# SHI-Labs/Versatile-Diffusion

Hardware: NVIDIA H100
Metric: 512x512 images/sec @ 50-step DDIM (bs=4/GPU) (higher is better)
Workload: dtype bf16

## Files before the change

### versatile-diffusion_b200/csrc/attention.cu

```cuda
#include "common.cuh"
#include "host_util.h"

namespace vdb {

constexpr int kBQ = 128;
constexpr float kRescaleThreshold = 8.0f;

struct alignas(64) AttnParams {
  CUtensorMap tmQ;
  CUtensorMap tmK;
  CUtensorMap tmV;
  int Nq, Nk;
  int q_bs, kv_bs;
  int q_col0, k_col0;
  int dv;
  int causal;
  float scale_log2;
  __nv_bfloat16* out;
  long long ldo;
};

template <int DK, int DVP, int BKV, int KV_STAGES>
constexpr size_t attention_smem_bytes() {
  return (DK / 64) * kBQ * 128 + KV_STAGES * ((DK / 64) * BKV * 128 + (BKV / 64) * DVP * 128) + (1 + 4 * KV_STAGES) * 8 + 1024;
}

template <int DK, int DVP, int BKV, int KV_STAGES>
__global__ void __launch_bounds__(288, 1) attention_kernel(const __grid_constant__ AttnParams p) {
  constexpr int KA = DK / 64;
  constexpr int KVA = BKV / 64;
  constexpr uint32_t kQBytes = KA * kBQ * 128;
  constexpr uint32_t kKBytes = KA * BKV * 128;
  constexpr uint32_t kVAtom = DVP * 128;
  constexpr uint32_t kVBytes = KVA * kVAtom;
  static_assert(BKV == 64 || BKV == 128, "kv tile");
  static_assert(kVAtom % 1024 == 0, "V atom must keep 1024B alignment");
  static_assert(DVP % 16 == 0 && DVP <= 256, "invalid wgmma N for PV");

  extern __shared__ __align__(1024) uint8_t smem_raw[];
  uint8_t* smem = reinterpret_cast<uint8_t*>((reinterpret_cast<uintptr_t>(smem_raw) + 1023) & ~uintptr_t(1023));
  uint8_t* sQ = smem;
  uint8_t* sK = sQ + kQBytes;
  uint8_t* sV = sK + KV_STAGES * kKBytes;
  uint64_t* q_full = reinterpret_cast<uint64_t*>(sV + KV_STAGES * kVBytes);
  uint64_t* k_full = q_full + 1;
  uint64_t* k_empty = k_full + KV_STAGES;
  uint64_t* v_full = k_empty + KV_STAGES;
  uint64_t* v_empty = v_full + KV_STAGES;

  const int warp = threadIdx.x >> 5;
  const int lane = threadIdx.x & 31;
  const int q0 = blockIdx.x * kBQ;
  const int head = blockIdx.y;
  const int b = blockIdx.z;

  int ntiles = (p.Nk + BKV - 1) / BKV;
  if (p.causal) ntiles = min(ntiles, (q0 + kBQ + BKV - 1) / BKV);

  if (warp == 8 && lane == 0) {
    tma_prefetch_desc(&p.tmQ);
    tma_prefetch_desc(&p.tmK);
    tma_prefetch_desc(&p.tmV);
  }
  if (threadIdx.x == 0) {
    mbar_init(q_full, 1);
    for (int s = 0; s < KV_STAGES; ++s) {
      mbar_init(&k_full[s], 1); mbar_init(&k_empty[s], 8);
      mbar_init(&v_full[s], 1); mbar_init(&v_empty[s], 8);
    }
    fence_barrier_init();
  }
  __syncthreads();
  pdl_launch_dependents();
  pdl_wait();

  if (warp == 8) {
    if (lane == 0) {
      mbar_arrive_expect_tx(q_full, kQBytes);
      for (int a = 0; a < KA; ++a)
        tma_load_2d(sQ + a * kBQ * 128, &p.tmQ, q_full, p.q_col0 + head * DK + a * 64, b * p.q_bs + q0);
      for (int j = 0; j < ntiles; ++j) {
        const int st = j % KV_STAGES;
        const uint32_t ph = (j / KV_STAGES) & 1;
        mbar_wait(&k_empty[st], ph ^ 1);
        mbar_arrive_expect_tx(&k_full[st], kKBytes);
        for (int a = 0; a < KA; ++a)
          tma_load_2d(sK + st * kKBytes + a * BKV * 128, &p.tmK, &k_full[st], p.k_col0 + head * DK + a * 64,
                      b * p.kv_bs + j * BKV);
        mbar_wait(&v_empty[st], ph ^ 1);
        mbar_arrive_expect_tx(&v_full[st], kVBytes);
        for (int a = 0; a < KVA; ++a)
          tma_load_2d(sV + st * kVBytes + a * kVAtom, &p.tmV, &v_full[st], b * p.kv_bs + j * BKV + a * 64, head * DVP);
      }
    }
    return;
  }

  const int g = warp >> 2;
  const int row0 = g * 64 + (warp & 3) * 16 + (lane >> 2);
  const int c2 = 2 * (lane & 3);
  const int q_idx[2] = {q0 + row0, q0 + row0 + 8};
  const int ksteps = (p.dv + 15) / 16;
  float o[DVP / 2];
#pragma unroll
  for (int i = 0; i < DVP / 2; ++i) o[i] = 0.f;
  float m_ref[2] = {-INFINITY, -INFINITY};
  float l_sum[2] = {0.f, 0.f};
  mbar_wait(q_full, 0);
#pragma unroll 1
  for (int j = 0; j < ntiles; ++j) {
    const int st = j % KV_STAGES;
    const uint32_t ph = (j / KV_STAGES) & 1;
    float s[BKV / 2];
    mbar_wait(&k_full[st], ph);
    wgmma_fence();
#pragma unroll
    for (int a = 0; a < KA; ++a) {
      const uint64_t qd = make_desc_sw128(smem_u32(sQ + a * kBQ * 128 + g * 64 * 128));
      const uint64_t kd = make_desc_sw128(smem_u32(sK + st * kKBytes + a * BKV * 128));
#pragma unroll
      for (int k = 0; k < 4; ++k)
        if (a * 4 + k < ksteps)
          wgmma_ss<BKV>(s, qd + 2 * k, kd + 2 * k, (a > 0 || k > 0) ? 1u : 0u);
    }
    wgmma_commit();
    wgmma_wait<0>();
    wgmma_fence_regs(s);
    __syncwarp();
    if (lane == 0) mbar_arrive(&k_empty[st]);

    const int kv0 = j * BKV;
    if (kv0 + BKV > p.Nk || p.causal) {
#pragma unroll
      for (int i = 0; i < 2; ++i) {
        const int lim = p.causal ? min(p.Nk, q_idx[i] + 1) : p.Nk;
#pragma unroll
        for (int jj = 0; jj < BKV / 8; ++jj)
#pragma unroll
          for (int e = 0; e < 2; ++e)
            if (kv0 + 8 * jj + c2 + e >= lim) s[4 * jj + 2 * i + e] = -INFINITY;
      }
    }
    float m_scaled[2];
#pragma unroll
    for (int i = 0; i < 2; ++i) {
      float mx = -INFINITY;
#pragma unroll
      for (int jj = 0; jj < BKV / 8; ++jj) mx = fmaxf(mx, fmaxf(s[4 * jj + 2 * i], s[4 * jj + 2 * i + 1]));
      mx = fmaxf(mx, __shfl_xor_sync(0xffffffffu, mx, 1));
      mx = fmaxf(mx, __shfl_xor_sync(0xffffffffu, mx, 2));
      const float m_new = fmaxf(m_ref[i], mx);
      if (j == 0 || m_ref[i] == -INFINITY) {
        m_ref[i] = m_new;
      } else if ((m_new - m_ref[i]) * p.scale_log2 > kRescaleThreshold) {
        const float factor = ex2_mufu((m_ref[i] - m_new) * p.scale_log2);
        m_ref[i] = m_new;
        l_sum[i] *= factor;
#pragma unroll
        for (int jj = 0; jj < DVP / 8; ++jj) {
          o[4 * jj + 2 * i] *= factor;
          o[4 * jj + 2 * i + 1] *= factor;
        }
      }
      m_scaled[i] = (m_ref[i] == -INFINITY) ? 0.f : m_ref[i] * p.scale_log2;
    }
    uint32_t pa[BKV / 16][4];
#pragma unroll
    for (int kk = 0; kk < BKV / 16; ++kk) {
#pragma unroll
      for (int h = 0; h < 4; ++h) {
        const int i = h & 1;
        const int idx = 8 * kk + 4 * (h >> 1) + 2 * i;
        const float e0 = ex2_mufu(fmaf(s[idx], p.scale_log2, -m_scaled[i]));
        const float e1 = ex2_mufu(fmaf(s[idx + 1], p.scale_log2, -m_scaled[i]));
        l_sum[i] += e0 + e1;
        pa[kk][h] = pack_bf16x2(e0, e1);
      }
    }
    mbar_wait(&v_full[st], ph);
    wgmma_fence();
#pragma unroll
    for (int kk = 0; kk < BKV / 16; ++kk) {
      const uint64_t vd = make_desc_sw128(smem_u32(sV + st * kVBytes + (kk >> 2) * kVAtom));
      wgmma_rs<DVP>(o, pa[kk], vd + 2 * (kk & 3), 1u);
    }
    wgmma_commit();
    wgmma_wait<0>();
    wgmma_fence_regs(o);
    __syncwarp();
    if (lane == 0) mbar_arrive(&v_empty[st]);
  }

#pragma unroll
  for (int i = 0; i < 2; ++i) {
    float l = l_sum[i];
    l += __shfl_xor_sync(0xffffffffu, l, 1);
    l += __shfl_xor_sync(0xffffffffu, l, 2);
    const float inv_l = 1.f / l;
    if (q_idx[i] >= p.Nq) continue;
    __nv_bfloat16* orow = p.out + (static_cast<long long>(b) * p.q_bs + q_idx[i]) * p.ldo + head * p.dv;
#pragma unroll
    for (int jj = 0; jj < DVP / 8; ++jj) {
      const int col = 8 * jj + c2;
      if (col < p.dv)
        *reinterpret_cast<uint32_t*>(orow + col) = pack_bf16x2(o[4 * jj + 2 * i] * inv_l, o[4 * jj + 2 * i + 1] * inv_l);
    }
  }
}

struct AttnArgs {
  const void *Q, *K, *Vt;
  long long ldq, ldk, ldv;
  int B, H, q_bstride, kv_bstride;
};

template <int DK, int DVP, int BKV, int KV_STAGES>
static int launch_attention(AttnParams& p, const AttnArgs& a, cudaStream_t stream) {
  constexpr size_t smem = attention_smem_bytes<DK, DVP, BKV, KV_STAGES>();
  static_assert(smem <= 227 * 1024, "attention smem budget");
  auto kernel = attention_kernel<DK, DVP, BKV, KV_STAGES>;
  static bool configured = false;
  if (!configured) {
    VDB_CUDA_CHECK(cudaFuncSetAttribute(kernel, cudaFuncAttributeMaxDynamicSharedMemorySize, static_cast<int>(smem)));
    prefer_max_smem(kernel);
    configured = true;
  }
  int rc = make_tmap_2d(&p.tmQ, a.Q, static_cast<uint64_t>(a.ldq), static_cast<uint64_t>(a.B) * a.q_bstride, a.ldq * 2, 64, kBQ);
  if (rc) return rc;
  rc = make_tmap_2d(&p.tmK, a.K, static_cast<uint64_t>(a.ldk), static_cast<uint64_t>(a.B) * a.kv_bstride, a.ldk * 2, 64, BKV);
  if (rc) return rc;
  rc = make_tmap_2d(&p.tmV, a.Vt, static_cast<uint64_t>(a.B) * a.kv_bstride, static_cast<uint64_t>(a.H) * DVP, a.ldv * 2, 64, DVP);
  if (rc) return rc;
  dim3 grid((p.Nq + kBQ - 1) / kBQ, a.H, a.B);
  VDB_CUDA_CHECK(launch_pdl(kernel, grid, dim3(288), smem, stream, p));
  count_launch();
  return VDB_OK;
}

}

using namespace vdb;

extern "C" {

int vdb_attention_dk_pad(int d_head) { return d_head <= 64 ? 64 : (d_head <= 128 ? 128 : (d_head <= 192 ? 192 : -1)); }
int vdb_attention_dv_pad(int d_head) {
  if (d_head <= 48) return 48;
  if (d_head <= 64) return 64;
  if (d_head <= 80) return 80;
  if (d_head <= 160) return 160;
  return -1;
}

int vdb_attention_bf16(const void* Q, long long ldq, int q_col0, const void* K, long long ldk, int k_col0,
                       const void* Vt, long long ldv, void* out, long long ldo, int B, int H, int Nq, int Nk,
                       int q_bstride, int kv_bstride, int d_head, float scale, int causal, void* stream) {
  if (!Q || !K || !Vt || !out || B <= 0 || H <= 0 || Nq <= 0 || Nk <= 0)
    return set_error(VDB_ERR_INVALID, "attention: null/empty argument");
  const int DK = vdb_attention_dk_pad(d_head), DVP = vdb_attention_dv_pad(d_head);
  if (DK < 0 || DVP < 0) return set_error(VDB_ERR_UNSUPPORTED, "attention: d_head %d not supported (<= 160)", d_head);
  if ((d_head % 8) || (ldo % 8) || (ldq % 8) || (ldk % 8) || (ldv % 8))
    return set_error(VDB_ERR_INVALID, "attention: d_head and leading dims must be multiples of 8");
  if (q_bstride <= 0) q_bstride = Nq;
  if (kv_bstride <= 0) kv_bstride = Nk;
  if (q_bstride < Nq || kv_bstride < Nk || (kv_bstride % 8))
    return set_error(VDB_ERR_INVALID, "attention: need q_bstride >= Nq, kv_bstride >= Nk and kv_bstride %% 8 == 0 (got %d, %d)",
                     q_bstride, kv_bstride);
  AttnParams p;
  memset(&p, 0, sizeof(p));
  const AttnArgs a{Q, K, Vt, ldq, ldk, ldv, B, H, q_bstride, kv_bstride};
  p.Nq = Nq; p.Nk = Nk; p.q_bs = q_bstride; p.kv_bs = kv_bstride; p.q_col0 = q_col0; p.k_col0 = k_col0; p.dv = d_head; p.causal = causal;
  p.scale_log2 = scale * 1.4426950408889634f;
  p.out = reinterpret_cast<__nv_bfloat16*>(out);
  p.ldo = ldo;
  cudaStream_t st = reinterpret_cast<cudaStream_t>(stream);
  if (DK == 64 && DVP == 48) return launch_attention<64, 48, 128, 2>(p, a, st);
  if (DK == 64 && DVP == 64) return launch_attention<64, 64, 128, 2>(p, a, st);
  if (DK == 128 && DVP == 80) return launch_attention<128, 80, 128, 2>(p, a, st);
  if (DK == 192 && DVP == 160) return launch_attention<192, 160, 64, 2>(p, a, st);
  return set_error(VDB_ERR_UNSUPPORTED, "attention: no kernel for d_head %d", d_head);
}

}
```

### versatile-diffusion_b200/csrc/common.cuh

```cuda
#pragma once
#include <cuda.h>
#include <cuda_bf16.h>
#include <cuda_runtime.h>
#include <stdint.h>

namespace vdb {

#define VDB_DEVINL __device__ __forceinline__

enum : int {
  VDB_OK = 0,
  VDB_ERR_INVALID = 1,
  VDB_ERR_CUDA = 2,
  VDB_ERR_UNSUPPORTED = 3,
};

VDB_DEVINL float4 lds_f4(uint32_t addr) {
  float4 v;
  asm volatile("ld.shared.v4.f32 {%0, %1, %2, %3}, [%4];" : "=f"(v.x), "=f"(v.y), "=f"(v.z), "=f"(v.w) : "r"(addr));
  return v;
}

VDB_DEVINL uint32_t smem_u32(const void* p) {
  return static_cast<uint32_t>(__cvta_generic_to_shared(p));
}

VDB_DEVINL uint32_t lane_id() {
  uint32_t l;
  asm volatile("mov.u32 %0, %%laneid;" : "=r"(l));
  return l;
}

VDB_DEVINL bool elect_one() {
  uint32_t pred = 0;
  asm volatile(
      "{\n\t"
      ".reg .pred P;\n\t"
      "elect.sync _|P, 0xffffffff;\n\t"
      "selp.u32 %0, 1, 0, P;\n\t"
      "}\n"
      : "=r"(pred));
  return pred != 0;
}

VDB_DEVINL void mbar_init(uint64_t* bar, uint32_t count) {
  asm volatile("mbarrier.init.shared::cta.b64 [%0], %1;" ::"r"(smem_u32(bar)), "r"(count));
}
VDB_DEVINL void fence_barrier_init() {
  asm volatile("fence.mbarrier_init.release.cluster;" ::: "memory");
}
VDB_DEVINL void fence_proxy_async_smem() {
  asm volatile("fence.proxy.async.shared::cta;" ::: "memory");
}
VDB_DEVINL void mbar_arrive_expect_tx(uint64_t* bar, uint32_t bytes) {
  asm volatile("mbarrier.arrive.expect_tx.shared::cta.b64 _, [%0], %1;" ::"r"(smem_u32(bar)),
               "r"(bytes)
               : "memory");
}
VDB_DEVINL void mbar_arrive(uint64_t* bar) {
  asm volatile("mbarrier.arrive.shared::cta.b64 _, [%0];" ::"r"(smem_u32(bar)) : "memory");
}
VDB_DEVINL bool mbar_try_wait(uint64_t* bar, uint32_t parity) {
  uint32_t ok;
  asm volatile(
      "{\n\t"
      ".reg .pred P;\n\t"
      "mbarrier.try_wait.parity.shared::cta.b64 P, [%1], %2;\n\t"
      "selp.u32 %0, 1, 0, P;\n\t"
      "}\n"
      : "=r"(ok)
      : "r"(smem_u32(bar)), "r"(parity)
      : "memory");
  return ok != 0;
}
VDB_DEVINL void mbar_wait(uint64_t* bar, uint32_t parity) {
  while (!mbar_try_wait(bar, parity)) {
  }
}

VDB_DEVINL void tma_prefetch_desc(const CUtensorMap* m) {
  asm volatile("prefetch.tensormap [%0];" ::"l"(reinterpret_cast<uint64_t>(m)) : "memory");
}
VDB_DEVINL void tma_load_2d(void* smem_dst, const CUtensorMap* m, uint64_t* bar, int c0, int c1) {
  asm volatile(
      "cp.async.bulk.tensor.2d.shared::cluster.global.tile.mbarrier::complete_tx::bytes"
      " [%0], [%1, {%3, %4}], [%2];" ::"r"(smem_u32(smem_dst)),
      "l"(reinterpret_cast<uint64_t>(m)), "r"(smem_u32(bar)), "r"(c0), "r"(c1)
      : "memory");
}
VDB_DEVINL void tma_load_4d(void* smem_dst, const CUtensorMap* m, uint64_t* bar, int c0, int c1,
                            int c2, int c3) {
  asm volatile(
      "cp.async.bulk.tensor.4d.shared::cluster.global.tile.mbarrier::complete_tx::bytes"
      " [%0], [%1, {%3, %4, %5, %6}], [%2];" ::"r"(smem_u32(smem_dst)),
      "l"(reinterpret_cast<uint64_t>(m)), "r"(smem_u32(bar)), "r"(c0), "r"(c1), "r"(c2), "r"(c3)
      : "memory");
}

VDB_DEVINL void tma_store_4d(const CUtensorMap* m, const void* smem_src, int c0, int c1, int c2, int c3) {
  asm volatile(
      "cp.async.bulk.tensor.4d.global.shared::cta.tile.bulk_group [%0, {%2, %3, %4, %5}], [%1];" ::"l"(
          reinterpret_cast<uint64_t>(m)),
      "r"(smem_u32(smem_src)), "r"(c0), "r"(c1), "r"(c2), "r"(c3)
      : "memory");
}
VDB_DEVINL void bulk_commit() { asm volatile("cp.async.bulk.commit_group;" ::: "memory"); }
template <int N>
VDB_DEVINL void bulk_wait_read() { asm volatile("cp.async.bulk.wait_group.read %0;" ::"n"(N) : "memory"); }
template <int N>
VDB_DEVINL void bulk_wait() { asm volatile("cp.async.bulk.wait_group %0;" ::"n"(N) : "memory"); }

VDB_DEVINL uint32_t cluster_ctarank() {
  uint32_t r;
  asm volatile("mov.u32 %0, %%cluster_ctarank;" : "=r"(r));
  return r;
}
VDB_DEVINL void cluster_sync_all() {
  asm volatile("barrier.cluster.arrive.release.aligned;\n\tbarrier.cluster.wait.acquire.aligned;" ::: "memory");
}
VDB_DEVINL uint32_t mapa_u32(uint32_t local_addr, uint32_t rank) {
  uint32_t r;
  asm volatile("mapa.shared::cluster.u32 %0, %1, %2;" : "=r"(r) : "r"(local_addr), "r"(rank));
  return r;
}
VDB_DEVINL void mbar_arrive_cluster(uint32_t cluster_addr) {
  asm volatile("mbarrier.arrive.release.cluster.shared::cluster.b64 _, [%0];" ::"r"(cluster_addr) : "memory");
}

VDB_DEVINL uint64_t make_desc_sw128(uint32_t smem_addr) {
  uint64_t d = 0;
  d |= static_cast<uint64_t>((smem_addr & 0x3FFFF) >> 4);
  d |= static_cast<uint64_t>(1) << 16;
  d |= static_cast<uint64_t>(1024 >> 4) << 32;
  d |= static_cast<uint64_t>(1) << 62;
  return d;
}
VDB_DEVINL void wgmma_fence() { asm volatile("wgmma.fence.sync.aligned;" ::: "memory"); }
VDB_DEVINL void wgmma_commit() { asm volatile("wgmma.commit_group.sync.aligned;" ::: "memory"); }
template <int N>
VDB_DEVINL void wgmma_wait() { asm volatile("wgmma.wait_group.sync.aligned %0;" ::"n"(N) : "memory"); }
template <int R>
VDB_DEVINL void wgmma_fence_regs(float (&d)[R]) {
#pragma unroll
  for (int i = 0; i < R; ++i) asm volatile("" : "+f"(d[i])::"memory");
}

VDB_DEVINL unsigned long long gtime() {
  unsigned long long t;
  asm volatile("mov.u64 %0, %%globaltimer;" : "=l"(t));
  return t;
}

VDB_DEVINL void pdl_wait() { asm volatile("griddepcontrol.wait;" ::: "memory"); }
VDB_DEVINL void pdl_launch_dependents() { asm volatile("griddepcontrol.launch_dependents;" ::: "memory"); }

VDB_DEVINL uint32_t pack_bf16x2(float lo, float hi) {
  __nv_bfloat162 v = __floats2bfloat162_rn(lo, hi);
  return *reinterpret_cast<uint32_t*>(&v);
}
VDB_DEVINL float2 unpack_bf16x2(uint32_t u) {
  __nv_bfloat162 v = *reinterpret_cast<__nv_bfloat162*>(&u);
  return __bfloat1622float2(v);
}
VDB_DEVINL float ex2_mufu(float x) {
  float y;
  asm("ex2.approx.ftz.f32 %0, %1;" : "=f"(y) : "f"(x));
  return y;
}
VDB_DEVINL float ex2_poly(float x) {
  x = fmaxf(x, -126.0f);
  const float r = x + 12582912.0f;
  const float f = x - (r - 12582912.0f);
  float p = fmaf(0.0550886838f, f, 0.242604051f);
  p = fmaf(p, f, 0.693276242f);
  p = fmaf(p, f, 0.99992894f);
  return __int_as_float(__float_as_int(p) + (__float_as_int(r) << 23));
}
VDB_DEVINL float silu_f(float x) { return __fdividef(x, 1.0f + __expf(-x)); }
VDB_DEVINL float silu_bf16_f(float x) {
  float th;
  asm("tanh.approx.f32 %0, %1;" : "=f"(th) : "f"(0.5f * x));
  const float hx = 0.5f * x;
  return fmaf(hx, th, hx);
}
VDB_DEVINL float gelu_erf_f(float x) { return 0.5f * x * (1.0f + erff(x * 0.70710678118654752f)); }
VDB_DEVINL float gelu_as_f(float x) {
  const float z = fabsf(x) * 0.70710678118654752f;
  const float t = __fdividef(1.0f, fmaf(0.3275911f, z, 1.0f));
  float poly = fmaf(1.061405429f, t, -1.453152027f);
  poly = fmaf(poly, t, 1.421413741f);
  poly = fmaf(poly, t, -0.284496736f);
  poly = fmaf(poly, t, 0.254829592f);
  const float erf_abs = 1.0f - poly * t * __expf(-z * z);
  return 0.5f * x * (1.0f + copysignf(erf_abs, x));
}
VDB_DEVINL float gelu_fast_f(float x) {
  const float u = x * fmaf(0.0356774081f, x * x, 0.7978845608f);
  float th;
  asm("tanh.approx.f32 %0, %1;" : "=f"(th) : "f"(u));
  const float hx = 0.5f * x;
  return fmaf(hx, th, hx);
}
VDB_DEVINL float quick_gelu_f(float x) { return __fdividef(x, 1.0f + __expf(-1.702f * x)); }

}

#include "wgmma.cuh"
```

Measured before the change: 3.412.

## Pipeline attention with producer warpgroup, register reallocation and ping-pong consumer scheduling

```diff
diff --git a/versatile-diffusion_b200/csrc/attention.cu b/versatile-diffusion_b200/csrc/attention.cu
--- a/versatile-diffusion_b200/csrc/attention.cu
+++ b/versatile-diffusion_b200/csrc/attention.cu
@@ -4,6 +4,8 @@
 namespace vdb {
 
 constexpr int kBQ = 128;
+constexpr int kAttnThreads = 384;
+constexpr int kTurnBar = 1;
 constexpr float kRescaleThreshold = 8.0f;
 
 struct alignas(64) AttnParams {
@@ -26,7 +28,7 @@
 }
 
 template <int DK, int DVP, int BKV, int KV_STAGES>
-__global__ void __launch_bounds__(288, 1) attention_kernel(const __grid_constant__ AttnParams p) {
+__global__ void __launch_bounds__(kAttnThreads, 1) attention_kernel(const __grid_constant__ AttnParams p) {
   constexpr int KA = DK / 64;
   constexpr int KVA = BKV / 64;
   constexpr uint32_t kQBytes = KA * kBQ * 128;
@@ -36,6 +38,8 @@
   static_assert(BKV == 64 || BKV == 128, "kv tile");
   static_assert(kVAtom % 1024 == 0, "V atom must keep 1024B alignment");
   static_assert(DVP % 16 == 0 && DVP <= 256, "invalid wgmma N for PV");
+  constexpr int kSSteps = DVP / 16;
+  static_assert(kSSteps <= 4 * KA, "DVP <= DK");
 
   extern __shared__ __align__(1024) uint8_t smem_raw[];
   uint8_t* smem = reinterpret_cast<uint8_t*>((reinterpret_cast<uintptr_t>(smem_raw) + 1023) & ~uintptr_t(1023));
@@ -57,7 +61,7 @@
   int ntiles = (p.Nk + BKV - 1) / BKV;
   if (p.causal) ntiles = min(ntiles, (q0 + kBQ + BKV - 1) / BKV);
 
-  if (warp == 8 && lane == 0) {
+  if (warp == 0 && lane == 0) {
     tma_prefetch_desc(&p.tmQ);
     tma_prefetch_desc(&p.tmK);
     tma_prefetch_desc(&p.tmV);
@@ -74,8 +78,9 @@
   pdl_launch_dependents();
   pdl_wait();
 
-  if (warp == 8) {
-    if (lane == 0) {
+  if (warp < 4) {
+    setmaxnreg_dec<24>();
+    if (warp == 0 && lane == 0) {
       mbar_arrive_expect_tx(q_full, kQBytes);
       for (int a = 0; a < KA; ++a)
         tma_load_2d(sQ + a * kBQ * 128, &p.tmQ, q_full, p.q_col0 + head * DK + a * 64, b * p.q_bs + q0);
@@ -95,40 +100,45 @@
     }
     return;
   }
-
-  const int g = warp >> 2;
+  setmaxnreg_inc<240>();
+
+  const int g = (warp >> 2) - 1;
   const int row0 = g * 64 + (warp & 3) * 16 + (lane >> 2);
   const int c2 = 2 * (lane & 3);
   const int q_idx[2] = {q0 + row0, q0 + row0 + 8};
-  const int ksteps = (p.dv + 15) / 16;
   float o[DVP / 2];
 #pragma unroll
   for (int i = 0; i < DVP / 2; ++i) o[i] = 0.f;
   float m_ref[2] = {-INFINITY, -INFINITY};
   float l_sum[2] = {0.f, 0.f};
-  mbar_wait(q_full, 0);
-#pragma unroll 1
-  for (int j = 0; j < ntiles; ++j) {
-    const int st = j % KV_STAGES;
-    const uint32_t ph = (j / KV_STAGES) & 1;
-    float s[BKV / 2];
-    mbar_wait(&k_full[st], ph);
-    wgmma_fence();
+  float s[BKV / 2];
+  uint32_t pa[BKV / 16][4], pb[BKV / 16][4];
+
+  auto issue_s = [&](int st) {
 #pragma unroll
     for (int a = 0; a < KA; ++a) {
       const uint64_t qd = make_desc_sw128(smem_u32(sQ + a * kBQ * 128 + g * 64 * 128));
       const uint64_t kd = make_desc_sw128(smem_u32(sK + st * kKBytes + a * BKV * 128));
 #pragma unroll
       for (int k = 0; k < 4; ++k)
-        if (a * 4 + k < ksteps)
+        if (a * 4 + k < kSSteps)
           wgmma_ss<BKV>(s, qd + 2 * k, kd + 2 * k, (a > 0 || k > 0) ? 1u : 0u);
     }
     wgmma_commit();
-    wgmma_wait<0>();
-    wgmma_fence_regs(s);
+  };
+  auto issue_pv = [&](int st, const uint32_t (&pin)[BKV / 16][4]) {
+#pragma unroll
+    for (int kk = 0; kk < BKV / 16; ++kk) {
+      const uint64_t vd = make_desc_sw128(smem_u32(sV + st * kVBytes + (kk >> 2) * kVAtom));
+      wgmma_rs<DVP>(o, pin[kk], vd + 2 * (kk & 3), 1u);
+    }
+    wgmma_commit();
+  };
+  auto release = [&](uint64_t* bar) {
     __syncwarp();
-    if (lane == 0) mbar_arrive(&k_empty[st]);
-
+    if (lane == 0) mbar_arrive(bar);
+  };
+  auto softmax = [&](int j, float (&factor)[2], uint32_t (&pout)[BKV / 16][4]) {
     const int kv0 = j * BKV;
     if (kv0 + BKV > p.Nk || p.causal) {
 #pragma unroll
@@ -144,27 +154,28 @@
     float m_scaled[2];
 #pragma unroll
     for (int i = 0; i < 2; ++i) {
-      float mx = -INFINITY;
-#pragma unroll
-      for (int jj = 0; jj < BKV / 8; ++jj) mx = fmaxf(mx, fmaxf(s[4 * jj + 2 * i], s[4 * jj + 2 * i + 1]));
+      factor[i] = 1.f;
+      float t[BKV / 8];
+#pragma unroll
+      for (int jj = 0; jj < BKV / 8; ++jj) t[jj] = fmaxf(s[4 * jj + 2 * i], s[4 * jj + 2 * i + 1]);
+#pragma unroll
+      for (int w = BKV / 16; w >= 1; w /= 2)
+#pragma unroll
+        for (int jj = 0; jj < BKV / 16; ++jj)
+          if (jj < w) t[jj] = fmaxf(t[jj], t[jj + w]);
+      float mx = t[0];
       mx = fmaxf(mx, __shfl_xor_sync(0xffffffffu, mx, 1));
       mx = fmaxf(mx, __shfl_xor_sync(0xffffffffu, mx, 2));
       const float m_new = fmaxf(m_ref[i], mx);
       if (j == 0 || m_ref[i] == -INFINITY) {
         m_ref[i] = m_new;
       } else if ((m_new - m_ref[i]) * p.scale_log2 > kRescaleThreshold) {
-        const float factor = ex2_mufu((m_ref[i] - m_new) * p.scale_log2);
+        factor[i] = ex2_mufu((m_ref[i] - m_new) * p.scale_log2);
         m_ref[i] = m_new;
-        l_sum[i] *= factor;
-#pragma unroll
-        for (int jj = 0; jj < DVP / 8; ++jj) {
-          o[4 * jj + 2 * i] *= factor;
-          o[4 * jj + 2 * i + 1] *= factor;
-        }
+        l_sum[i] *= factor[i];
       }
       m_scaled[i] = (m_ref[i] == -INFINITY) ? 0.f : m_ref[i] * p.scale_log2;
     }
-    uint32_t pa[BKV / 16][4];
 #pragma unroll
     for (int kk = 0; kk < BKV / 16; ++kk) {
 #pragma unroll
@@ -174,22 +185,69 @@
         const float e0 = ex2_mufu(fmaf(s[idx], p.scale_log2, -m_scaled[i]));
         const float e1 = ex2_mufu(fmaf(s[idx + 1], p.scale_log2, -m_scaled[i]));
         l_sum[i] += e0 + e1;
-        pa[kk][h] = pack_bf16x2(e0, e1);
-      }
-    }
-    mbar_wait(&v_full[st], ph);
+        pout[kk][h] = pack_bf16x2(e0, e1);
+      }
+    }
+  };
+
+  const int my_turn = kTurnBar + g, other_turn = kTurnBar + (g ^ 1);
+  if (g == 1) named_bar_arrive(other_turn, 256);
+  mbar_wait(q_full, 0);
+
+  float factor[2];
+  named_bar_sync(my_turn, 256);
+  mbar_wait(&k_full[0], 0);
+  wgmma_fence();
+  issue_s(0);
+  named_bar_arrive(other_turn, 256);
+  wgmma_wait<0>();
+  wgmma_fence_regs(s);
+  release(&k_empty[0]);
+  softmax(0, factor, pa);
+  auto step = [&](int j, const uint32_t (&pin)[BKV / 16][4], uint32_t (&pout)[BKV / 16][4]) {
+    const int st = j % KV_STAGES, pst = (j - 1) % KV_STAGES;
+    named_bar_sync(my_turn, 256);
+    mbar_wait(&k_full[st], (j / KV_STAGES) & 1);
     wgmma_fence();
-#pragma unroll
-    for (int kk = 0; kk < BKV / 16; ++kk) {
-      const uint64_t vd = make_desc_sw128(smem_u32(sV + st * kVBytes + (kk >> 2) * kVAtom));
-      wgmma_rs<DVP>(o, pa[kk], vd + 2 * (kk & 3), 1u);
-    }
-    wgmma_commit();
+    issue_s(st);
+    mbar_wait(&v_full[pst], ((j - 1) / KV_STAGES) & 1);
+    issue_pv(pst, pin);
+    named_bar_arrive(other_turn, 256);
+    wgmma_wait<1>();
+    wgmma_fence_regs(s);
+    release(&k_empty[st]);
+    softmax(j, factor, pout);
     wgmma_wait<0>();
     wgmma_fence_regs(o);
-    __syncwarp();
-    if (lane == 0) mbar_arrive(&v_empty[st]);
-  }
+    release(&v_empty[pst]);
+#pragma unroll
+    for (int i = 0; i < 2; ++i)
+      if (factor[i] < 1.f) {
+#pragma unroll
+        for (int jj = 0; jj < DVP / 8; ++jj) {
+          o[4 * jj + 2 * i] *= factor[i];
+          o[4 * jj + 2 * i + 1] *= factor[i];
+        }
+      }
+  };
+  int j = 1;
+#pragma unroll 1
+  for (; j + 1 < ntiles; j += 2) {
+    step(j, pa, pb);
+    step(j + 1, pb, pa);
+  }
+  if (j < ntiles) step(j, pa, pb);
+  const int lst = (ntiles - 1) % KV_STAGES;
+  mbar_wait(&v_full[lst], ((ntiles - 1) / KV_STAGES) & 1);
+  wgmma_fence();
+  if (ntiles & 1)
+    issue_pv(lst, pa);
+  else
+    issue_pv(lst, pb);
+  wgmma_wait<0>();
+  wgmma_fence_regs(o);
+  release(&v_empty[lst]);
+  if (g == 0) named_bar_sync(my_turn, 256);
 
 #pragma unroll
   for (int i = 0; i < 2; ++i) {
@@ -232,7 +290,7 @@
   rc = make_tmap_2d(&p.tmV, a.Vt, static_cast<uint64_t>(a.B) * a.kv_bstride, static_cast<uint64_t>(a.H) * DVP, a.ldv * 2, 64, DVP);
   if (rc) return rc;
   dim3 grid((p.Nq + kBQ - 1) / kBQ, a.H, a.B);
-  VDB_CUDA_CHECK(launch_pdl(kernel, grid, dim3(288), smem, stream, p));
+  VDB_CUDA_CHECK(launch_pdl(kernel, grid, dim3(kAttnThreads), smem, stream, p));
   count_launch();
   return VDB_OK;
 }
diff --git a/versatile-diffusion_b200/csrc/common.cuh b/versatile-diffusion_b200/csrc/common.cuh
--- a/versatile-diffusion_b200/csrc/common.cuh
+++ b/versatile-diffusion_b200/csrc/common.cuh
@@ -144,6 +144,14 @@
 #pragma unroll
   for (int i = 0; i < R; ++i) asm volatile("" : "+f"(d[i])::"memory");
 }
+
+template <int N>
+VDB_DEVINL void setmaxnreg_dec() { asm volatile("setmaxnreg.dec.sync.aligned.u32 %0;" ::"n"(N)); }
+template <int N>
+VDB_DEVINL void setmaxnreg_inc() { asm volatile("setmaxnreg.inc.sync.aligned.u32 %0;" ::"n"(N)); }
+
+VDB_DEVINL void named_bar_sync(int id, int threads) { asm volatile("bar.sync %0, %1;" ::"r"(id), "r"(threads) : "memory"); }
+VDB_DEVINL void named_bar_arrive(int id, int threads) { asm volatile("bar.arrive %0, %1;" ::"r"(id), "r"(threads) : "memory"); }
 
 VDB_DEVINL unsigned long long gtime() {
   unsigned long long t;
```

New measurement: 3.444 (median of 6 runs). About the same (+1.0%).
